# rainerzufalldererste/limg

Measured on AMD Instinct MI355X. Metric: encode Mpixels/s, 8K RGBA (limg_encode3d_test-equivalent: all 11 planes stored), higher is better.
Workload: dtype u8/i32 integer stage + f32 float stage (bit-exact vs the reference's strict SSE build)

## Files before the change

### limg_amd/csrc/limg_hip_device.h

```cpp
#ifndef LIMG_HIP_DEVICE_H
#define LIMG_HIP_DEVICE_H

#include "limg_hip_wave.h"
#include "limg_rsqrt_x86_table.h"

#include <float.h>

namespace limg_hip
{
  namespace
  {
    __device__ __attribute__((aligned(16))) const unsigned short d_rsqrt_x86_tab[2048] = LIMG_RSQRT_X86_TAB_INIT;

    enum : uint32_t { kZeroA = 1u, kZeroB = 2u, kZeroC = 4u, kValid = 8u };

    template <int CTRL, int ROWMASK>
    __device__ __forceinline__ int dpp(int oldv, int v) { return __builtin_amdgcn_update_dpp(oldv, v, CTRL, ROWMASK, 0xF, false); }

    __device__ __forceinline__ uint32_t wave_sum(uint32_t x)
    {
      int v = (int)x;
      v += dpp<0xB1, 0xF>(0, v);
      v += dpp<0x4E, 0xF>(0, v);
      v += dpp<0x141, 0xF>(0, v);
      v += dpp<0x140, 0xF>(0, v);
      v += dpp<0x142, 0xA>(0, v);
      v += dpp<0x143, 0xC>(0, v);
      return (uint32_t)__builtin_amdgcn_readlane(v, 63);
    }

    __device__ __forceinline__ int sgpr(int v) { return __builtin_amdgcn_readfirstlane(v); }
    __device__ __forceinline__ float sgprf(float v) { return __int_as_float(__builtin_amdgcn_readfirstlane(__float_as_int(v))); }

    template <int CH>
    __device__ __forceinline__ float dpps(const float a[4], const float b[4])
    {
      const float p0 = a[0] * b[0], p1 = a[1] * b[1], p2 = a[2] * b[2];
      const float p3 = CH == 4 ? a[3] * b[3] : 0.0f;
      return (p0 + p1) + (p2 + p3);
    }

    __device__ __forceinline__ void px_to_float(uint32_t px, float f[4])
    {
      f[0] = (float)(px & 0xFF); f[1] = (float)((px >> 8) & 0xFF); f[2] = (float)((px >> 16) & 0xFF); f[3] = (float)(px >> 24);
    }

    __device__ __forceinline__ int cvt_rne(float x) { return (int)__builtin_rintf(x); }
    __device__ __forceinline__ uint32_t cvt_u8_rne_sat(float x) { uint32_t r; asm("v_cvt_pk_u8_f32 %0, %1, 0, 0" : "=v"(r) : "v"(x)); return r; }

    __device__ __forceinline__ void store_v(float *V, int lane, const float v[4])
    {
      *reinterpret_cast<float4 *>(V + lane * 4) = make_float4(v[0], v[1], v[2], v[3]);
    }

    struct RecU
    {
      int nA[3], nB[3], nC[3], mA[3], mB[3], mC[3];
    };

    __device__ __forceinline__ uint32_t trial_error(const uint32_t px, const uint32_t fA, const uint32_t fB, const uint32_t fC, const RecU &r, const uint32_t sA,
                                                    const uint32_t sB, const uint32_t sC)
    {
      const uint32_t dA = (fA >> sA) * shift_mul(sA), dB = (fB >> sB) * shift_mul(sB), dC = (fC >> sC) * shift_mul(sC);
      uint32_t dsq[3];
#pragma unroll
      for (int c = 0; c < 3; c++)
      {
        const int nA = sA > 7 ? 0 : r.nA[c], nB = sB > 7 ? 0 : r.nB[c], nC = sC > 7 ? 0 : r.nC[c];
        const int mA = r.mA[c], mB = sB > 7 ? 128 : r.mB[c], mC = sC > 7 ? 128 : r.mC[c];
        int est = ((int)(dA * (uint32_t)nA + (uint32_t)mA) >> 8) + ((int)(dB * (uint32_t)nB + (uint32_t)mB) >> 8) + ((int)(dC * (uint32_t)nC + (uint32_t)mC) >> 8);
        est = est < 0 ? 0 : (est > 255 ? 255 : est);
        const int d = (int)((px >> (8 * c)) & 0xFF) - est;
        dsq[c] = (uint32_t)(d * d);
      }
      const bool low_red = (int)dsq[0] < 0x4000;
      return dsq[0] * (low_red ? 2u : 3u) + dsq[2] * (low_red ? 3u : 2u) + dsq[1] * 4u;
    }

    __device__ __forceinline__ bool trial(const uint32_t px, const uint32_t fA, const uint32_t fB, const uint32_t fC, const RecU &r, const uint32_t sA,
                                          const uint32_t sB, const uint32_t sC, const bool active, const uint32_t maxPixel32, const uint64_t maxBlockN,
                                          uint32_t &blockError)
// ... 291 lines not shown
```

### limg_amd/csrc/limg_hip_encode.hip

```cpp
#include "limg_hip_context.h"
#include "limg_search_table_accurate.h"

using namespace limg_hip;

namespace limg_hip
{
  Partition partition(size_t sizeY, int poolThreads)
  {
    Partition pt = { 1, 0 };
    if (poolThreads <= 0) return pt;
    size_t thread_count = (size_t)poolThreads * 4;
    size_t y_range = ((sizeY / kBlock) / thread_count) * kBlock;
    if (y_range == 0)
    {
      thread_count = (size_t)poolThreads;
      y_range = ((sizeY / kBlock) / thread_count) * kBlock;
    }
    if (y_range == 0) return pt;
    pt.chainCount = (uint32_t)thread_count;
    pt.chainRows = (uint32_t)(y_range / kBlock);
    return pt;
  }

  limg_hip_result encode_stats(const EncodeJob &e)
// ... 38 lines not shown
      e[5] = mul[a]; e[6] = mul[b]; e[7] = mul[cc];
    }
    static_assert((size_t)LIMG_SEARCH_ACC_STATES * 32u < (1u << 24), "offsets leave bits 24..26 free");
    for (size_t i = 0; i < (size_t)LIMG_SEARCH_ACC_STATES; i++)
    {
      uint32_t *e = &wide[i * 8];
      if (e[0] >> 31) continue;
      for (int k = 1; k <= 2; k++)
      {
        const uint32_t *n = &wide[(e[k] / 32u) * 8];
        uint32_t mask = 0;
        if (!(n[0] >> 31)) mask = ((n[0] & 31u) != (e[0] & 31u) ? 1u : 0u) | (n[3] != e[3] ? 2u : 0u) | (n[4] != e[4] ? 4u : 0u);
        e[k] |= mask << 24;
      }
    }
    limg_hip_result r = c->accTable.ensure(wide.size() * 4);
    if (r != limg_hip_success) return r;
    if (hipMemcpy(c->accTable.p, wide.data(), wide.size() * 4, hipMemcpyHostToDevice) != hipSuccess) { c->accTable.release(); return limg_hip_error_Generic; }
    return limg_hip_success;
  }

  limg_hip_result ensure_pipe_events(limg_hip_context *c, size_t n)
  {
    if (!c->fitStream) HIP_TRY(hipStreamCreateWithFlags(&c->fitStream, hipStreamNonBlocking));
    while (c->pipeEvents.size() < n)
    {
      hipEvent_t e;
      HIP_TRY(hipEventCreateWithFlags(&e, hipEventDisableTiming));
      c->pipeEvents.push_back(e);
    }
    return limg_hip_success;
  }

  limg_hip_result encode_height_ragged(limg_hip_context *c, const uint32_t *dIn, size_t sizeX, size_t sizeY, int hasAlpha, const limg_hip_encode3d_info *dInfo,
                                       const limg_hip_compact_out *compact, uint32_t errorFactor, int poolThreads, int fast, hipStream_t stream, const EncodeExtra &x);

  limg_hip_result encode_params(EncodeJob &e, const uint32_t *dIn, const limg_hip_compact_out *compact, uint32_t errorFactor, int poolThreads, int fast)
  {
    limg_hip_context *const c = e.c;
    const EncodeExtra &x = e.x;
    const limg_hip_encode3d_info *const dInfo = e.dInfo;
    const size_t sizeX = e.sizeX, sizeY = e.sizeY, batchCount = x.batchCount;
    const ImageIO *const batch = x.batch;
    EncodeParams &p = e.p;
    memset(&p, 0, sizeof(p));
    p.io.in = dIn;
    p.sizeX = (uint32_t)sizeX; p.sizeY = (uint32_t)sizeY;
    p.blocksX = (uint32_t)((sizeX + kBlock - 1) / kBlock);
    p.blocksY = (uint32_t)((sizeY + kBlock - 1) / kBlock);
    p.stripsX = (p.blocksX + kStripBlocks - 1) / kStripBlocks;
    const uint64_t maxPixel = (uint64_t)0x6 * (errorFactor / 2) * 7, maxBlock = (uint64_t)0x4 * (errorFactor / 2) * 7;
    p.maxPixel32 = maxPixel > 0xFFFFFFFFull ? 0xFFFFFFFFu : (uint32_t)maxPixel;
    p.maxBlock = maxBlock;
    { const uint64_t lim = (maxBlock * 64ull + 15ull) >> 4; p.blockLimitFull = lim > 0xFFFFFFFFull ? 0xFFFFFFFFu : (uint32_t)lim; }
    p.crushBits = errorFactor != 0;
    p.fast = fast != 0;
    p.accTable = nullptr;
    if (!p.fast && p.crushBits)
    {
      limg_hip_result ra = ensure_accurate_table(c);
      if (ra != limg_hip_success) return ra;
      p.accTable = (const uint32_t *)c->accTable.p;
    }
    const bool forced = c->opt.forced_shift[0] >= 0 && c->opt.forced_shift[0] <= 8 && c->opt.forced_shift[1] >= 0 && c->opt.forced_shift[1] <= 8 &&
                        c->opt.forced_shift[2] >= 0 && c->opt.forced_shift[2] <= 8;
    for (int i = 0; i < 3; i++) p.forced[i] = forced ? c->opt.forced_shift[i] : -1;
    p.floatFast = (c->opt.float_mode == 1 && !x.fitOnly) ? 1 : 0;
    p.recordLimit = TOPT(c, record_limit) > 0 ? TOPT(c, record_limit) - 1 : 2700;
    const Partition pt = e.pt = x.part ? *x.part : partition(sizeY, poolThreads);
    p.chainCount = pt.chainCount; p.chainRows = pt.chainRows;

    p.batchCount = (uint32_t)batchCount;
    p.imageStrips = p.stripsX * p.blocksY;
    e.blocks = (size_t)p.blocksX * p.blocksY * batchCount; e.strips = (size_t)p.stripsX * p.blocksY * batchCount;
    const size_t scratchRows = x.scratchRows > (size_t)p.blocksY * batchCount ? x.scratchRows : (size_t)p.blocksY * batchCount;
    const size_t scratchBlocks = scratchRows * p.blocksX, scratchStrips = scratchRows * p.stripsX;
    const size_t blockOff = x.scratchRow0 * p.blocksX, stripOff = x.scratchRow0 * p.stripsX;
    limg_hip_result r;
    if (compact && compact->pRecords) p.records = compact->pRecords + blockOff;
    else { if ((r = c->records.ensure(scratchBlocks * sizeof(limg_hip_block_record))) != limg_hip_success) return r; p.records = (limg_hip_block_record *)c->records.p + blockOff; }
    if (compact && compact->pShifts) p.shifts = compact->pShifts + blockOff;
    else { if ((r = c->shifts.ensure(scratchBlocks * 4)) != limg_hip_success) return r; p.shifts = (uint32_t *)c->shifts.p + blockOff; }
    if ((r = c->invN.ensure(scratchBlocks * 16)) != limg_hip_success) return r;
    p.invN = (float *)c->invN.p + blockOff * 4;
    if ((r = c->stripCalls.ensure(scratchStrips * 4)) != limg_hip_success) return r;
    if ((r = c->stripBase.ensure(scratchStrips * 4)) != limg_hip_success) return r;
    p.stripCalls = (uint32_t *)c->stripCalls.p + stripOff; p.stripBase = (uint32_t *)c->stripBase.p + stripOff;
    const bool fullPlanes = e.fullPlanes;
    p.storePlanes = dInfo != nullptr;
    p.fullPlanes = fullPlanes;
    p.streamRaw = x.streamRaw && !fullPlanes;
    p.stripWords = (x.streamRaw && !fullPlanes) ? x.stripWords : nullptr;
    p.fitOnly = x.fitOnly && !dInfo;
    if (dInfo) p.io.info = *dInfo;
    p.vecIn = (sizeX % 4 == 0) && (((uintptr_t)dIn) & 15u) == 0;
    p.vecPlanes = 0;
    if (dInfo && fullPlanes && sizeX % 4 == 0)
    {
      uintptr_t bits = 0;
      const void *const *pp = reinterpret_cast<const void *const *>(dInfo);
      for (int i = 1; i < 8; i++) bits |= (uintptr_t)pp[i];
      p.vecPlanes = (bits & 15u) == 0;
    }
    p.vecFactors8 = dInfo && (sizeX % 8 == 0) && ((((uintptr_t)dInfo->pFactorsA) | ((uintptr_t)dInfo->pFactorsB) | ((uintptr_t)dInfo->pFactorsC)) & 7u) == 0;
    p.vecDecoded = dInfo && fullPlanes && (sizeX % 4 == 0) && (((uintptr_t)dInfo->pDecoded) & 15u) == 0;
    p.vecFactors = dInfo && (sizeX % 16 == 0) && ((((uintptr_t)dInfo->pFactorsA) | ((uintptr_t)dInfo->pFactorsB) | ((uintptr_t)dInfo->pFactorsC)) & 15u) == 0;
    if (batchCount > 1)
// ... 384 lines not shown
```

### limg_amd/csrc/limg_hip_internal.h

```cpp
#ifndef LIMG_HIP_INTERNAL_H
#define LIMG_HIP_INTERNAL_H

#include <hip/hip_runtime.h>
#include <stdint.h>

#include <type_traits>

#include "../../include/limg_hip.h"
#include "limg_hip_blocked_host.h"

namespace limg_hip
{
  constexpr int kBlock = 8;
  constexpr int kStripBlocks = 32;
  constexpr int kThreads = 256;
  constexpr int kWaves = 4;
  constexpr int kBlocksPerWave = 8;
  constexpr uint64_t kDitherSeed = 0xCA7F00D15BADF00DULL;

  struct ImageIO
  {
    const uint32_t *in;
    limg_hip_encode3d_info info;
  };

  struct EncodeParams
  {
    ImageIO io;
    const ImageIO *batch;
    uint32_t batchCount, imageStrips;
    uint32_t sizeX, sizeY, blocksX, blocksY, stripsX;
    uint32_t maxPixel32;
    uint64_t maxBlock;
    uint32_t blockLimitFull;
    int32_t crushBits, fast;
    const uint32_t *accTable;
    int32_t forced[3];
    int32_t recordLimit;
    uint32_t chainCount, chainRows;
    limg_hip_block_record *records;
    float *invN;
    uint32_t *shifts;
    uint32_t *stripCalls;
    uint32_t *stripBase;
    uint32_t *stripWords;
    int32_t storePlanes;
    int32_t fullPlanes;
    const uint8_t *noise;
    uint32_t noiseLast;
    unsigned long long *desc;
    uint32_t *ticket;
    int32_t zeroLookback;
    uint32_t *timeout;
#ifdef LIMG_HIP_TEST_HOOKS
    uint32_t lookbackSpins;
    uint32_t testBaseErrStrip;
    uint32_t testSkipStrip;
#endif
    uint8_t *park;
    int32_t compactOut;
    int32_t streamRaw;
    int32_t fitOnly;
    unsigned long long *chainCallsOut;
    const unsigned long long *chainBase;
    int32_t fitPrio;
    int32_t prefit;
    int32_t floatFast;
    int32_t vecIn;
    int32_t vecPlanes;
    int32_t vecFactors;
    int32_t vecFactors8;
    int32_t vecDecoded;
  };

  struct StreamParams
  {
    uint32_t sizeX, sizeY, blocksX, blocksY, nBlocks, nTiles, channels, errorFactor, flags;
    const uint8_t *fac[3];
    const limg_hip_block_record *records;
    const uint32_t *shifts;
    uint8_t *stream;
    uint32_t *tileBase;
    uint32_t *stripWords;
    uint32_t stripsX, nStrips, nWaves;
  };

  struct StreamImage
  {
// ... 163 lines not shown
```

### limg_amd/csrc/limg_hip_kernels.hip

```cpp
#include "limg_hip_search.h"
#include "limg_hip_phase_f.h"
#include "limg_hip_float_pixel.h"
#include "limg_hip_lookback.h"

namespace limg_hip
{
  namespace
  {
    constexpr int kPrioE = 2;


    constexpr int kLdsStrip = 0, kLdsV = kLdsStrip + 8 * kRowDw * 4, kLdsVBytes = kWaves * kBatch * kVDw * 4;
    constexpr int kLdsBlk = kLdsV + kLdsVBytes, kLdsCalls = kLdsBlk + kStripBlocks * 192, kLdsTotal = kLdsCalls + 32;
    static_assert(kLdsTotal <= 32768 - 16, "5 workgroups per CU");
    struct LdsLayout { int v, blk, calls, trialc, total; };
    constexpr int kTrialConstDw = 20;
    template <bool PREFIT> __device__ __host__ constexpr LdsLayout lds_layout()
    {
      if (!PREFIT) return LdsLayout{ kLdsV, kLdsBlk, kLdsCalls, kLdsV, kLdsTotal };
      const int v = kLdsStrip + 8 * kRowDw * 4, blk = v + kFacBytes, calls = blk + kStripBlocks * 192, tc = calls + 32, e = tc + kStripBlocks * kTrialConstDw * 4;
      const int f = kLdsStrip + kPhaseFBytes + kStripBlocks * 48 + 16;
      return LdsLayout{ v, blk, calls, tc, e > f ? e : f };
    }
    static_assert(lds_layout<true>().total <= 163840 / 6, "6 workgroups per CU with the float stage in its own kernel");
// ... 354 lines not shown
      uint32_t *s_queue = s_calls + 4;
      if (tid == 0) *s_queue = 0;
      __syncthreads();

      uint8_t *stage = reinterpret_cast<uint8_t *>(s_V);
      uint32_t waveCalls = 0;

      auto grab = [&]() -> uint32_t { uint32_t v = 0; if (lane == 0) v = atomicAdd(s_queue, 1u); return (uint32_t)sgpr((int)v); };
      uint32_t sbNext = grab();
#pragma unroll 1
      for (;;)
      {
        const uint32_t sb = sbNext;
        if (sb >= (uint32_t)kStripBlocks) break;
        uint32_t qv = 0;
        if (lane == 0) qv = atomicAdd(s_queue, 1u);
        const uint32_t bx = strip * kStripBlocks + sb;
        if (bx >= p.blocksX) { sbNext = (uint32_t)sgpr((int)qv); continue; }
        const uint32_t rx = min(p.sizeX - bx * kBlock, (uint32_t)kBlock), n = rx * ry;
        BlkF *const blkE = s_blk + sb;
        uint32_t lx, ly;
        if (rx == 8) { lx = lane & 7; ly = lane >> 3; }
        else { const uint32_t l = (uint32_t)lane < n ? (uint32_t)lane : 0u; ly = l / rx; lx = l - ly * rx; }
        uint32_t px = s_strip[ly * kRowDw + sb * kBlock + lx];
        const bool active = (uint32_t)lane < n;
        px = active ? px : 0u;
        const BlkE *be = reinterpret_cast<const BlkE *>(blkE);

        uint32_t fA, fB, fC;
        {
          const V4 pv = px_to_v4(px);
          const V4 nA = ld4(be->nrm[0]), mnA = ld4(be->off[0]);
          const float fa = dp4<CH, FAST>(pv - mnA, nA) * be->invN[0];
          fA = cvt_u8_rne_sat(255.0f * fa);
          const V4 nB = ld4(be->nrm[1]), ofB = ld4(be->off[1]);
          V4 est = mnA + nA * fa;
          const float fb = dp4<CH, FAST>((pv - est) - ofB, nB) * be->invN[1];
          fB = cvt_u8_rne_sat(255.0f * fb);
          const V4 nC = ld4(be->nrm[2]), ofC = ld4(be->off[2]);
          est = est + nB * fb;
          const float fc = dp4<CH, FAST>((pv - est) - ofC, nC) * be->invN[2];
          fC = cvt_u8_rne_sat(255.0f * fc);
        }

        uint32_t shift[3] = { 0, 0, 0 };
        if (p.forced[0] >= 0)
        {
          shift[0] = (uint32_t)p.forced[0]; shift[1] = (uint32_t)p.forced[1]; shift[2] = (uint32_t)p.forced[2];
        }
        else if (p.crushBits)
        {
          const uint64_t maxBlockN = p.maxBlock * (uint64_t)n;
          uint32_t blockLimit = p.blockLimitFull;
          if (n != 64)
          {
            const uint64_t lim64 = (maxBlockN + 15ull) >> 4;
            blockLimit = (uint32_t)sgpr((int)(lim64 > 0xFFFFFFFFull ? 0xFFFFFFFFu : (uint32_t)lim64));
          }
          const bool big = ((uint32_t)sgpr((int)blkE->flags) & kBig) != 0;
          if (!big)
          {
            TrialState t;
            t.fA = fA; t.fB = fB; t.fC = fC;
            const uint32_t R = px & 0xFF, G = (px >> 8) & 0xFF;
            t.hiRG = (R + 0x8000u) | ((G + 0x8000u) << 16);
            t.loRG = (R + 0x8000u - 255u) | ((G + 0x8000u - 255u) << 16);
            t.pxB = (int)((px >> 16) & 0xFF);
            t.pxBlo = t.pxB - 255;
            if (PREFIT)
            {
              const int *tc = s_trialc + sb * kTrialConstDw;
#pragma unroll
              for (int c = 0; c < 3; c++)
              {
                t.nA[c] = tc[c]; t.nB[c] = tc[3 + c]; t.nC[c] = tc[6 + c];
                t.mA[c] = tc[9 + c]; t.mB[c] = tc[12 + c]; t.mC[c] = tc[15 + c];
              }
            }
            else
            {
#pragma unroll
              for (int c = 0; c < 3; c++)
              {
                const int loA = blkE->rec[c], hiA = blkE->rec[4 + c], loB = blkE->rec[8 + c], hiB = blkE->rec[12 + c], loC = blkE->rec[16 + c], hiC = blkE->rec[20 + c];
                t.nA[c] = loA - hiA; t.nB[c] = loB - hiB; t.nC[c] = loC - hiC;
                t.mA[c] = term_const(0, c, loA); t.mB[c] = term_const(1, c, loB); t.mC[c] = term_const(2, c, loC);
              }
            }
            t.mA[0] += (int)(R << 8); t.mA[1] += (int)(G << 8); t.mA[2] += t.pxB << 8;
            if (!ACC)
            {
              if (n == 64) search_fast_automaton<true>(t, true, p.maxPixel32, blockLimit, shift);
              else search_fast_automaton<false>(t, active, p.maxPixel32, blockLimit, shift);
            }
            else
            {
              if (n == 64) search_accurate_automaton<true>(t, true, p.maxPixel32, blockLimit, p.accTable, shift);
              else search_accurate_automaton<false>(t, active, p.maxPixel32, blockLimit, p.accTable, shift);
            }
          }
          else
          {
            const uint32_t packed = (uint32_t)sgpr((int)search_generic(px, fA, fB, fC, blkE->rec, active, p.maxPixel32, maxBlockN, !ACC));
            shift[0] = packed & 0xFF; shift[1] = (packed >> 8) & 0xFF; shift[2] = (packed >> 16) & 0xFF;
          }
        }

        const uint32_t calls = (((shift[0] & 7u) + 7u) >> 3) + (((shift[1] & 7u) + 7u) >> 3) + (((shift[2] & 7u) + 7u) >> 3);
        waveCalls += calls;
        if (p.stripWords)
        {
          uint32_t words = 0;
#pragma unroll
          for (int k = 0; k < 3; k++)
          {
            const uint32_t sk = shift[k];
            if (sk < 8u) words += 8u - sk;
            else if (CH == 4 && sgpr((int)blkE->rec[8 * k + 3]) != sgpr((int)blkE->rec[8 * k + 7])) words += 8u;
          }
          waveCalls += words << 8;
        }

        const size_t bi = (size_t)byS * p.blocksX + bx;
        const uint32_t word = shift[0] | (shift[1] << 8) | (shift[2] << 16) | (calls << 24);
        if (lane == 0)
        {
          if (!PERSIST || p.compactOut) p.shifts[bi] = word;
          if (PERSIST) reinterpret_cast<uint32_t *>(park + kParkShift)[sb] = word;
        }
        if (p.storePlanes && active)
        {
          const uint32_t o = ly * kFacRow + sb * kBlock + lx;
          stage[o] = (uint8_t)fA; stage[kFacPlane + o] = (uint8_t)fB; stage[2 * kFacPlane + o] = (uint8_t)fC;
        }
        sbNext = (uint32_t)sgpr((int)qv);
      }
      if (lane == 0) s_calls[wave] = waveCalls;
      __syncthreads();
      if (tid == 0)
      {
        const uint32_t aggAll = s_calls[0] + s_calls[1] + s_calls[2] + s_calls[3];
        const uint32_t agg = aggAll & 0xFFu;
        if (p.stripWords) p.stripWords[id] = aggAll >> 8;
        if (PERSIST)
        {
          uint32_t headId = head0;
// ... 337 lines not shown
```

### limg_amd/csrc/limg_hip_search.h

```cpp
#ifndef LIMG_HIP_SEARCH_H
#define LIMG_HIP_SEARCH_H

#include "limg_hip_device.h"
#include "limg_search_table.h"

namespace limg_hip
{
  namespace
  {
    struct __attribute__((aligned(32))) SearchEntry { uint32_t w[8]; };
    __constant__ SearchEntry d_search_tab[LIMG_SEARCH_STATES] = LIMG_SEARCH_TABLE_INIT;

    typedef short short2_t __attribute__((ext_vector_type(2)));
    typedef unsigned short ushort2_t __attribute__((ext_vector_type(2)));
    __device__ __forceinline__ constexpr int term_bias(int factor) { return factor == 2 ? 0x2000 : 0x3000; }
    __device__ __forceinline__ int term_const(int f, int c, int lo) { return 255 - ((lo << 8) + 128) + (c < 2 ? (term_bias(f) << 8) : 0); }

    struct TrialState
    {
      uint32_t fA, fB, fC;
      uint32_t loRG, hiRG;
      int pxB, pxBlo;
      int nA[3], nB[3], nC[3];
      int mA[3], mB[3], mC[3];
// ... 25 lines not shown
    }

    template <bool FULL>
    __device__ __forceinline__ uint32_t trial_pixel_error(const TrialState &t, const bool active)
    {
      const uint32_t dRG = t.tA_RG + t.tB_RG + t.tC_RG;
      const int dBraw = t.tA_B + t.tB_B + t.tC_B;
      ushort2_t eu = __builtin_bit_cast(ushort2_t, dRG);
      eu = __builtin_elementwise_max(eu, __builtin_bit_cast(ushort2_t, t.loRG));
      eu = __builtin_elementwise_min(eu, __builtin_bit_cast(ushort2_t, t.hiRG));
      int dB = med3_i32(dBraw, t.pxBlo, t.pxB);
      const ushort2_t sq = eu * eu;
      const uint32_t sqB = (uint32_t)mul_i24(dB, dB);
      const bool low_red = sq.x < 0x4000;
      const uint32_t half = __builtin_amdgcn_udot2(sq, __builtin_bit_cast(ushort2_t, 0x00020001u), sqB, false);
      const uint32_t extra = low_red ? sqB : (__builtin_bit_cast(uint32_t, sq) & 0xFFFFu);
      uint32_t err = (half << 1) + extra;
      if (!FULL) err = active ? err : 0u;
      return err;
    }

    typedef unsigned int uint8s_t __attribute__((ext_vector_type(8)));
    __device__ __forceinline__ uint8s_t sload8(const SearchEntry *base, uint32_t byteOffset)
    {
      uint8s_t v;
      asm volatile("s_load_dwordx8 %0, %1, %2\n\ts_waitcnt lgkmcnt(0)" : "=&s"(v) : "s"(base), "s"(byteOffset) : "memory");
      return v;
    }

    struct TermSet { uint32_t rg; int b; };
    __device__ __forceinline__ constexpr TermSet terms_shift8(int factor) { return TermSet{ (uint32_t)term_bias(factor) * 0x10001u, 0 }; }
    template <uint32_t S, uint32_t MUL>
    __device__ __forceinline__ TermSet hot_terms(const uint32_t f, const int n[3], const int m[3])
    {
      static_assert(S <= 8 && (S >= 4 || MUL == (1u << S)), "MUL is shift_mul(S)");
      int t0, t1, t2;
      if constexpr (S == 8) { t0 = m[0]; t1 = m[1]; t2 = m[2]; }
      else
      {
        uint32_t d;
        if constexpr (S < 4) d = f & ~((1u << S) - 1u);
        else asm("v_mul_u32_u24 %0, %2, %1" : "=v"(d) : "v"(f >> S), "n"(MUL));
        t0 = mad_i24((int)d, n[0], m[0]); t1 = mad_i24((int)d, n[1], m[1]); t2 = mad_i24((int)d, n[2], m[2]);
      }
      TermSet r;
      r.rg = __builtin_amdgcn_perm((uint32_t)t1, (uint32_t)t0, 0x06050201u);
      r.b = t2 >> 8;
      return r;
    }
    __device__ __forceinline__ bool hot_trial(TrialState &t, const TermSet &A, const TermSet &B, const TermSet &C, const uint32_t maxPixel32, const uint32_t blockLimit)
    {
      t.tA_RG = A.rg; t.tA_B = A.b; t.tB_RG = B.rg; t.tB_B = B.b; t.tC_RG = C.rg; t.tC_B = C.b;
      const uint32_t err = trial_pixel_error<true>(t, true);
      return __builtin_amdgcn_ballot_w64(err > maxPixel32) == 0ull && wave_sum(err) < blockLimit;
    }
#include "limg_search_hot.h"

    template <bool FULL>
    __device__ __forceinline__ void search_fast_automaton(TrialState &t, const bool active, const uint32_t maxPixel32, const uint32_t blockLimit, uint32_t shift[3])
    {
      const SearchEntry *tab = d_search_tab;
      uint8s_t e;
      if constexpr (FULL)
      {
        uint32_t off;
        if (search_hot(t, maxPixel32, blockLimit, shift, off)) return;
        asm volatile("" : "+s"(tab));
        e = sload8(tab, off);
      }
      else
      {
        asm volatile("" : "+s"(tab));
        constexpr uint32_t root[8] = LIMG_SEARCH_ROOT;
        rebuild_A(t, root[0] & 31u, root[5]);
        rebuild_B(t, root[3], root[6]);
        rebuild_C(t, root[4], root[7]);
        e = uint8s_t{ root[0] & ~0xE0u, root[1], root[2], root[3], root[4], root[5], root[6], root[7] };
      }
      while (!(e[0] >> 31))
      {
        if (e[0] & 0x20u) rebuild_A(t, e[0] & 31u, e[5]);
        if (e[0] & 0x40u) rebuild_B(t, e[3], e[6]);
        if (e[0] & 0x80u) rebuild_C(t, e[4], e[7]);
        const uint32_t err = trial_pixel_error<FULL>(t, active);
        uint32_t off;
        if (__builtin_amdgcn_ballot_w64(err > maxPixel32) != 0ull) off = e[2];
        else off = (wave_sum(err) < blockLimit) ? e[1] : e[2];
        e = sload8(tab, off);
      }
      shift[0] = e[0] & 31u; shift[1] = e[3]; shift[2] = e[4];
    }

    template <bool FULL>
    __device__ __forceinline__ void search_accurate_automaton(TrialState &t, const bool active, const uint32_t maxPixel32, const uint32_t blockLimit, const uint32_t *table,
                                                              uint32_t shift[3])
    {
      const SearchEntry *tab = reinterpret_cast<const SearchEntry *>(table);
      uint32_t bestA = 0, bestB = 0, bestC = 0, minBe = 0xFFFFFFFFu;
      {
        constexpr uint32_t root[8] = LIMG_SEARCH_ROOT;
        rebuild_A(t, root[0] & 31u, root[5]);
        rebuild_B(t, root[3], root[6]);
        rebuild_C(t, root[4], root[7]);
      }
      uint8s_t e = sload8(tab, 0u);
      constexpr uint32_t rootT[8] = LIMG_SEARCH_ROOT;
      uint32_t mask = ((e[0] & 31u) != (rootT[0] & 31u) ? 1u : 0u) | (e[3] != rootT[3] ? 2u : 0u) | (e[4] != rootT[4] ? 4u : 0u);
      while (!(e[0] >> 31))
      {
        const uint32_t a = e[0] & 31u;
        if (mask & 1u) rebuild_A(t, a, e[5]);
        if (mask & 2u) rebuild_B(t, e[3], e[6]);
        if (mask & 4u) rebuild_C(t, e[4], e[7]);
        const uint32_t err = trial_pixel_error<FULL>(t, active);
        uint32_t off = e[2];
        if (__builtin_amdgcn_ballot_w64(err > maxPixel32) == 0ull)
        {
          const uint32_t be = wave_sum(err);
          if (be < blockLimit)
          {
            off = e[1];
            if (!(e[0] & 0x20u) || be < minBe) { bestA = a; bestB = e[3]; bestC = e[4]; minBe = be; }
          }
        }
        mask = off >> 24;
        e = sload8(tab, off & 0xFFFFFFu);
      }
      shift[0] = bestA; shift[1] = bestB; shift[2] = bestC;
    }

    __device__ __attribute__((noinline)) uint32_t search_generic(uint32_t px, uint32_t fA, uint32_t fB, uint32_t fC, const int16_t *rec , bool active,
                                                                 uint32_t maxPixel32, uint64_t maxBlockN, bool fast)
    {
      RecU r;
#pragma unroll
      for (int c = 0; c < 3; c++)
      {
        const int loA = rec[c], hiA = rec[4 + c], loB = rec[8 + c], hiB = rec[12 + c], loC = rec[16 + c], hiC = rec[20 + c];
        r.nA[c] = sgpr(hiA - loA); r.nB[c] = sgpr(hiB - loB); r.nC[c] = sgpr(hiC - loC);
        r.mA[c] = sgpr((int)(((uint32_t)loA << 8) + 128u)); r.mB[c] = sgpr((int)(((uint32_t)loB << 8) + 128u)); r.mC[c] = sgpr((int)(((uint32_t)loC << 8) + 128u));
// ... 12 lines not shown
```

### limg_amd/csrc/limg_search_hot.h

```cpp
#ifndef LIMG_SEARCH_HOT_H
#define LIMG_SEARCH_HOT_H
#define LIMG_SEARCH_HOT_STATES 45
__device__ __forceinline__ bool search_hot(TrialState &t, const uint32_t maxPixel32, const uint32_t blockLimit, uint32_t shift[3], uint32_t &off)
{
  const TermSet tA4_0 = hot_terms<4u, 17u>(t.fA, t.nA, t.mA);
  const TermSet tB5_0 = hot_terms<5u, 36u>(t.fB, t.nB, t.mB);
  const TermSet tC6_0 = hot_terms<6u, 85u>(t.fC, t.nC, t.mC);
  if (hot_trial(t, tA4_0, tB5_0, tC6_0, maxPixel32, blockLimit))
  {
    const TermSet tA5_1 = hot_terms<5u, 36u>(t.fA, t.nA, t.mA);
    if (hot_trial(t, tA5_1, terms_shift8(1), terms_shift8(2), maxPixel32, blockLimit))
    { shift[0] = 5u; shift[1] = 8u; shift[2] = 8u; return true; }
    else
    {
      const TermSet tB6_3 = hot_terms<6u, 85u>(t.fB, t.nB, t.mB);
      if (hot_trial(t, tA4_0, tB6_3, terms_shift8(2), maxPixel32, blockLimit))
      {
        if (hot_trial(t, tA4_0, terms_shift8(1), terms_shift8(2), maxPixel32, blockLimit))
        { t.cA = 4u; t.cB = 8u; t.cC = 8u; off = 0x00a0u; return false; }
        else
        {
          const TermSet tA6_23 = hot_terms<6u, 85u>(t.fA, t.nA, t.mA);
          if (hot_trial(t, tA6_23, tB6_3, terms_shift8(2), maxPixel32, blockLimit))
          {
            if (hot_trial(t, tA6_23, terms_shift8(1), terms_shift8(2), maxPixel32, blockLimit))
            { t.cA = 6u; t.cB = 8u; t.cC = 8u; off = 0x00c0u; return false; }
            else
            {
              const TermSet tA8_25 = hot_terms<8u, 256u>(t.fA, t.nA, t.mA);
              if (hot_trial(t, tA8_25, tB6_3, terms_shift8(2), maxPixel32, blockLimit))
              { t.cA = 8u; t.cB = 6u; t.cC = 8u; off = 0x0180u; return false; }
              else
              {
                if (hot_trial(t, tA8_25, terms_shift8(1), tC6_0, maxPixel32, blockLimit))
                { t.cA = 8u; t.cB = 8u; t.cC = 6u; off = 0x0220u; return false; }
                else
                {
                  const TermSet tB7_27 = hot_terms<7u, 255u>(t.fB, t.nB, t.mB);
                  if (hot_trial(t, tA6_23, tB7_27, terms_shift8(2), maxPixel32, blockLimit))
                  { t.cA = 6u; t.cB = 7u; t.cC = 8u; off = 0x0380u; return false; }
                  else
                  {
                    const TermSet tA7_31 = hot_terms<7u, 255u>(t.fA, t.nA, t.mA);
                    if (hot_trial(t, tA7_31, tB6_3, terms_shift8(2), maxPixel32, blockLimit))
                    { t.cA = 7u; t.cB = 6u; t.cC = 8u; off = 0x0400u; return false; }
                    else
                    { shift[0] = 6u; shift[1] = 6u; shift[2] = 8u; return true; }
                  }
                }
              }
            }
          }
          else
          {
            if (hot_trial(t, tA6_23, terms_shift8(1), tC6_0, maxPixel32, blockLimit))
            { t.cA = 6u; t.cB = 8u; t.cC = 6u; off = 0x0480u; return false; }
            else
            {
              const TermSet tA8_47 = hot_terms<8u, 256u>(t.fA, t.nA, t.mA);
              if (hot_trial(t, tA8_47, tB6_3, terms_shift8(2), maxPixel32, blockLimit))
              { t.cA = 8u; t.cB = 6u; t.cC = 8u; off = 0x0180u; return false; }
              else
              {
                if (hot_trial(t, tA8_47, terms_shift8(1), tC6_0, maxPixel32, blockLimit))
                { t.cA = 8u; t.cB = 8u; t.cC = 6u; off = 0x0220u; return false; }
                else
                {
                  const TermSet tB7_49 = hot_terms<7u, 255u>(t.fB, t.nB, t.mB);
                  if (hot_trial(t, tA4_0, tB7_49, terms_shift8(2), maxPixel32, blockLimit))
                  { t.cA = 4u; t.cB = 7u; t.cC = 8u; off = 0x0640u; return false; }
                  else
                  {
                    if (hot_trial(t, tA5_1, tB6_3, terms_shift8(2), maxPixel32, blockLimit))
                    {
                      if (hot_trial(t, tA5_1, tB7_49, terms_shift8(2), maxPixel32, blockLimit))
                      { shift[0] = 5u; shift[1] = 7u; shift[2] = 8u; return true; }
                      else
                      { shift[0] = 5u; shift[1] = 6u; shift[2] = 8u; return true; }
                    }
                    else
                    { shift[0] = 4u; shift[1] = 6u; shift[2] = 8u; return true; }
                  }
                }
              }
            }
          }
        }
      }
      else
      {
        if (hot_trial(t, tA4_0, tB5_0, terms_shift8(2), maxPixel32, blockLimit))
        { t.cA = 4u; t.cB = 5u; t.cC = 8u; off = 0x0740u; return false; }
        else
        {
          const TermSet tB7_96 = hot_terms<7u, 255u>(t.fB, t.nB, t.mB);
          const TermSet tC5_96 = hot_terms<5u, 36u>(t.fC, t.nC, t.mC);
          if (hot_trial(t, tA4_0, tB7_96, tC5_96, maxPixel32, blockLimit))
          { t.cA = 4u; t.cB = 7u; t.cC = 5u; off = 0x0c20u; return false; }
          else
          {
            const TermSet tA6_112 = hot_terms<6u, 85u>(t.fA, t.nA, t.mA);
            const TermSet tB4_112 = hot_terms<4u, 17u>(t.fB, t.nB, t.mB);
            const TermSet tC7_112 = hot_terms<7u, 255u>(t.fC, t.nC, t.mC);
            if (hot_trial(t, tA6_112, tB4_112, tC7_112, maxPixel32, blockLimit))
            { t.cA = 6u; t.cB = 4u; t.cC = 7u; off = 0x0c60u; return false; }
            else
            {
              const TermSet tC4_113 = hot_terms<4u, 17u>(t.fC, t.nC, t.mC);
              if (hot_trial(t, tA6_112, tB6_3, tC4_113, maxPixel32, blockLimit))
              { t.cA = 6u; t.cB = 6u; t.cC = 4u; off = 0x0e40u; return false; }
              else
              {
                if (hot_trial(t, tA6_112, terms_shift8(1), tC6_0, maxPixel32, blockLimit))
                { t.cA = 6u; t.cB = 8u; t.cC = 6u; off = 0x0480u; return false; }
                else
                {
                  const TermSet tA8_138 = hot_terms<8u, 256u>(t.fA, t.nA, t.mA);
                  if (hot_trial(t, tA8_138, tB6_3, terms_shift8(2), maxPixel32, blockLimit))
                  { t.cA = 8u; t.cB = 6u; t.cC = 8u; off = 0x0180u; return false; }
                  else
                  {
                    if (hot_trial(t, tA8_138, terms_shift8(1), tC6_0, maxPixel32, blockLimit))
                    { t.cA = 8u; t.cB = 8u; t.cC = 6u; off = 0x0220u; return false; }
                    else
                    {
                      if (hot_trial(t, tA4_0, tB5_0, tC7_112, maxPixel32, blockLimit))
                      { t.cA = 4u; t.cB = 5u; t.cC = 7u; off = 0x11a0u; return false; }
                      else
                      {
                        if (hot_trial(t, tA5_1, tB5_0, tC6_0, maxPixel32, blockLimit))
                        {
                          if (hot_trial(t, tA5_1, tB5_0, tC7_112, maxPixel32, blockLimit))
                          { shift[0] = 5u; shift[1] = 5u; shift[2] = 7u; return true; }
                          else
                          { shift[0] = 5u; shift[1] = 5u; shift[2] = 6u; return true; }
                        }
                        else
                        { shift[0] = 4u; shift[1] = 5u; shift[2] = 6u; return true; }
                      }
                    }
                  }
                }
              }
            }
          }
        }
      }
    }
  }
  else
  {
    const TermSet tA2_148 = hot_terms<2u, 4u>(t.fA, t.nA, t.mA);
    const TermSet tB4_148 = hot_terms<4u, 17u>(t.fB, t.nB, t.mB);
    const TermSet tC5_148 = hot_terms<5u, 36u>(t.fC, t.nC, t.mC);
    if (hot_trial(t, tA2_148, tB4_148, tC5_148, maxPixel32, blockLimit))
    {
      const TermSet tC7_149 = hot_terms<7u, 255u>(t.fC, t.nC, t.mC);
      if (hot_trial(t, tA2_148, tB4_148, tC7_149, maxPixel32, blockLimit))
      { t.cA = 2u; t.cB = 4u; t.cC = 7u; off = 0x12c0u; return false; }
      else
      {
        const TermSet tB6_378 = hot_terms<6u, 85u>(t.fB, t.nB, t.mB);
        const TermSet tC4_378 = hot_terms<4u, 17u>(t.fC, t.nC, t.mC);
        if (hot_trial(t, tA2_148, tB6_378, tC4_378, maxPixel32, blockLimit))
        { t.cA = 2u; t.cB = 6u; t.cC = 4u; off = 0x2f60u; return false; }
        else
        {
          if (hot_trial(t, tA2_148, terms_shift8(1), tC6_0, maxPixel32, blockLimit))
          { t.cA = 2u; t.cB = 8u; t.cC = 6u; off = 0x18e0u; return false; }
          else
          {
            const TermSet tB2_412 = hot_terms<2u, 4u>(t.fB, t.nB, t.mB);
            if (hot_trial(t, tA4_0, tB2_412, terms_shift8(2), maxPixel32, blockLimit))
            { t.cA = 4u; t.cB = 2u; t.cC = 8u; off = 0x2500u; return false; }
            else
            {
              if (hot_trial(t, tA4_0, tB4_148, tC4_378, maxPixel32, blockLimit))
              {
                if (hot_trial(t, tA4_0, tB4_148, tC6_0, maxPixel32, blockLimit))
                { t.cA = 4u; t.cB = 4u; t.cC = 6u; off = 0x2700u; return false; }
                else
                {
                  if (hot_trial(t, tA4_0, tB6_378, tC4_378, maxPixel32, blockLimit))
                  { t.cA = 4u; t.cB = 6u; t.cC = 4u; off = 0x2a40u; return false; }
                  else
                  {
                    if (hot_trial(t, tA4_0, terms_shift8(1), tC6_0, maxPixel32, blockLimit))
                    { t.cA = 4u; t.cB = 8u; t.cC = 6u; off = 0x1460u; return false; }
                    else
                    {
                      const TermSet tA6_417 = hot_terms<6u, 85u>(t.fA, t.nA, t.mA);
                      if (hot_trial(t, tA6_417, tB4_148, terms_shift8(2), maxPixel32, blockLimit))
                      { t.cA = 6u; t.cB = 4u; t.cC = 8u; off = 0x1620u; return false; }
                      else
                      {
                        if (hot_trial(t, tA6_417, tB6_378, tC4_378, maxPixel32, blockLimit))
                        { t.cA = 6u; t.cB = 6u; t.cC = 4u; off = 0x0e40u; return false; }
                        else
                        {
                          if (hot_trial(t, tA6_417, terms_shift8(1), tC6_0, maxPixel32, blockLimit))
                          { t.cA = 6u; t.cB = 8u; t.cC = 6u; off = 0x0480u; return false; }
                          else
                          {
                            const TermSet tA8_420 = hot_terms<8u, 256u>(t.fA, t.nA, t.mA);
                            if (hot_trial(t, tA8_420, tB6_378, terms_shift8(2), maxPixel32, blockLimit))
                            { t.cA = 8u; t.cB = 6u; t.cC = 8u; off = 0x0180u; return false; }
                            else
                            {
                              if (hot_trial(t, tA8_420, terms_shift8(1), tC6_0, maxPixel32, blockLimit))
                              { t.cA = 8u; t.cB = 8u; t.cC = 6u; off = 0x0220u; return false; }
                              else
                              {
                                if (hot_trial(t, tA4_0, tB4_148, tC5_148, maxPixel32, blockLimit))
                                {
                                  if (hot_trial(t, tA4_0, tB5_0, tC5_148, maxPixel32, blockLimit))
                                  {
                                    const TermSet tA5_424 = hot_terms<5u, 36u>(t.fA, t.nA, t.mA);
                                    if (hot_trial(t, tA5_424, tB5_0, tC5_148, maxPixel32, blockLimit))
                                    { shift[0] = 5u; shift[1] = 5u; shift[2] = 5u; return true; }
                                    else
                                    { shift[0] = 4u; shift[1] = 5u; shift[2] = 5u; return true; }
                                  }
                                  else
                                  {
                                    const TermSet tA5_427 = hot_terms<5u, 36u>(t.fA, t.nA, t.mA);
                                    if (hot_trial(t, tA5_427, tB4_148, tC5_148, maxPixel32, blockLimit))
                                    { t.cA = 5u; t.cB = 4u; t.cC = 5u; off = 0x3580u; return false; }
                                    else
                                    {
                                      if (hot_trial(t, tA5_427, tB5_0, tC4_378, maxPixel32, blockLimit))
                                      { t.cA = 5u; t.cB = 5u; t.cC = 4u; off = 0x35e0u; return false; }
                                      else
                                      { shift[0] = 4u; shift[1] = 4u; shift[2] = 5u; return true; }
                                    }
                                  }
                                }
                                else
                                { t.cA = 4u; t.cB = 4u; t.cC = 5u; off = 0x3640u; return false; }
                              }
                            }
                          }
                        }
                      }
                    }
                  }
                }
              }
              else
              { t.cA = 4u; t.cB = 4u; t.cC = 4u; off = 0x3780u; return false; }
            }
          }
        }
      }
    }
    else
    { t.cA = 2u; t.cB = 4u; t.cC = 5u; off = 0x3880u; return false; }
  }
}
#endif
```

Measured before the change: 54590.

## Add ballot-count early-reject screens before wave sum in hot search trials

Adds a cheap pre-screen to many hot-path search trials. It counts the lanes whose error meets a per-K threshold (limit/K) with a ballot and popcount, and rejects the trial when K or more lanes exceed it, since their sum must then reach the limit. This aims to skip the DPP reduction on failing trials. Separately, the wave-sum comparison now uses a ballot on lane 63 instead of readlane. The screen adds extra ballots and popcounts on trials that pass, and its benefit depends on how often the trials that were screened actually fail.

```diff
diff --git a/limg_amd/csrc/limg_hip_device.h b/limg_amd/csrc/limg_hip_device.h
--- a/limg_amd/csrc/limg_hip_device.h
+++ b/limg_amd/csrc/limg_hip_device.h
@@ -27,6 +27,20 @@
       v += dpp<0x142, 0xA>(0, v);
       v += dpp<0x143, 0xC>(0, v);
       return (uint32_t)__builtin_amdgcn_readlane(v, 63);
+    }
+
+    __device__ __forceinline__ bool wave_sum_below(uint32_t x, uint32_t limit)
+    {
+      int v = (int)x;
+      v += dpp<0xB1, 0xF>(0, v);
+      v += dpp<0x4E, 0xF>(0, v);
+      v += dpp<0x141, 0xF>(0, v);
+      v += dpp<0x140, 0xF>(0, v);
+      v += dpp<0x142, 0xA>(0, v);
+      v += dpp<0x143, 0xC>(0, v);
+      uint32_t hi = (uint32_t)(__builtin_amdgcn_ballot_w64((uint32_t)v < limit) >> 32);
+      asm volatile("" : "+s"(hi));
+      return (int32_t)hi < 0;
     }
 
     __device__ __forceinline__ int sgpr(int v) { return __builtin_amdgcn_readfirstlane(v); }
diff --git a/limg_amd/csrc/limg_hip_encode.hip b/limg_amd/csrc/limg_hip_encode.hip
--- a/limg_amd/csrc/limg_hip_encode.hip
+++ b/limg_amd/csrc/limg_hip_encode.hip
@@ -114,7 +114,8 @@
     const uint64_t maxPixel = (uint64_t)0x6 * (errorFactor / 2) * 7, maxBlock = (uint64_t)0x4 * (errorFactor / 2) * 7;
     p.maxPixel32 = maxPixel > 0xFFFFFFFFull ? 0xFFFFFFFFu : (uint32_t)maxPixel;
     p.maxBlock = maxBlock;
-    { const uint64_t lim = (maxBlock * 64ull + 15ull) >> 4; p.blockLimitFull = lim > 0xFFFFFFFFull ? 0xFFFFFFFFu : (uint32_t)lim; }
+    p.blockLimitFull = block_sum_limit(maxBlock, 64);
+    for (int i = 0; i < 4; i++) p.sumScreenT[i] = sum_screen_threshold(p.blockLimitFull, 8u << i);
     p.crushBits = errorFactor != 0;
     p.fast = fast != 0;
     p.accTable = nullptr;
diff --git a/limg_amd/csrc/limg_hip_internal.h b/limg_amd/csrc/limg_hip_internal.h
--- a/limg_amd/csrc/limg_hip_internal.h
+++ b/limg_amd/csrc/limg_hip_internal.h
@@ -8,6 +8,7 @@
 
 #include "../../include/limg_hip.h"
 #include "limg_hip_blocked_host.h"
+#include "limg_hip_sum_screen.h"
 
 namespace limg_hip
 {
@@ -34,6 +35,7 @@
     uint64_t maxBlock;
     uint32_t blockLimitFull;
     int32_t crushBits, fast;
+    uint32_t sumScreenT[4];
     const uint32_t *accTable;
     int32_t forced[3];
     int32_t recordLimit;
diff --git a/limg_amd/csrc/limg_hip_kernels.hip b/limg_amd/csrc/limg_hip_kernels.hip
--- a/limg_amd/csrc/limg_hip_kernels.hip
+++ b/limg_amd/csrc/limg_hip_kernels.hip
@@ -430,11 +430,7 @@
         {
           const uint64_t maxBlockN = p.maxBlock * (uint64_t)n;
           uint32_t blockLimit = p.blockLimitFull;
-          if (n != 64)
-          {
-            const uint64_t lim64 = (maxBlockN + 15ull) >> 4;
-            blockLimit = (uint32_t)sgpr((int)(lim64 > 0xFFFFFFFFull ? 0xFFFFFFFFu : (uint32_t)lim64));
-          }
+          if (n != 64) blockLimit = (uint32_t)sgpr((int)block_sum_limit(p.maxBlock, n));
           const bool big = ((uint32_t)sgpr((int)blkE->flags) & kBig) != 0;
           if (!big)
           {
@@ -468,8 +464,9 @@
             t.mA[0] += (int)(R << 8); t.mA[1] += (int)(G << 8); t.mA[2] += t.pxB << 8;
             if (!ACC)
             {
-              if (n == 64) search_fast_automaton<true>(t, true, p.maxPixel32, blockLimit, shift);
-              else search_fast_automaton<false>(t, active, p.maxPixel32, blockLimit, shift);
+              const uint32_t sumT[4] = { p.sumScreenT[0], p.sumScreenT[1], p.sumScreenT[2], p.sumScreenT[3] };
+              if (n == 64) search_fast_automaton<true>(t, true, p.maxPixel32, blockLimit, sumT, shift);
+              else search_fast_automaton<false>(t, active, p.maxPixel32, blockLimit, sumT, shift);
             }
             else
             {
diff --git a/limg_amd/csrc/limg_hip_search.h b/limg_amd/csrc/limg_hip_search.h
--- a/limg_amd/csrc/limg_hip_search.h
+++ b/limg_amd/csrc/limg_hip_search.h
@@ -101,19 +101,49 @@
     {
       t.tA_RG = A.rg; t.tA_B = A.b; t.tB_RG = B.rg; t.tB_B = B.b; t.tC_RG = C.rg; t.tC_B = C.b;
       const uint32_t err = trial_pixel_error<true>(t, true);
-      return __builtin_amdgcn_ballot_w64(err > maxPixel32) == 0ull && wave_sum(err) < blockLimit;
+      return __builtin_amdgcn_ballot_w64(err > maxPixel32) == 0ull && wave_sum_below(err, blockLimit);
+    }
+    __device__ __forceinline__ uint32_t lane_count(const uint64_t mask) { uint32_t c; asm("s_bcnt1_i32_b64 %0, %1" : "=s"(c) : "s"(mask) : "scc"); return c; }
+    template <int K>
+    __device__ __forceinline__ bool sum_screen(const uint32_t err, const uint32_t TK) { return lane_count(__builtin_amdgcn_ballot_w64(err >= TK)) >= (uint32_t)K; }
+    template <int K>
+    __device__ __forceinline__ bool hot_trial_after(TrialState &t, const TermSet &A, const TermSet &B, const TermSet &C, const uint32_t maxPixel32, const uint32_t blockLimit,
+                                                    const uint32_t TK)
+    {
+      t.tA_RG = A.rg; t.tA_B = A.b; t.tB_RG = B.rg; t.tB_B = B.b; t.tC_RG = C.rg; t.tC_B = C.b;
+      const uint32_t err = trial_pixel_error<true>(t, true);
+      return __builtin_amdgcn_ballot_w64(err > maxPixel32) == 0ull && !sum_screen<K>(err, TK) && wave_sum_below(err, blockLimit);
+    }
+    template <int K>
+    __device__ __forceinline__ bool hot_trial_first(TrialState &t, const TermSet &A, const TermSet &B, const TermSet &C, const uint32_t maxPixel32, const uint32_t blockLimit,
+                                                    const uint32_t TK)
+    {
+      t.tA_RG = A.rg; t.tA_B = A.b; t.tB_RG = B.rg; t.tB_B = B.b; t.tC_RG = C.rg; t.tC_B = C.b;
+      const uint32_t err = trial_pixel_error<true>(t, true);
+      return !sum_screen<K>(err, TK) && __builtin_amdgcn_ballot_w64(err > maxPixel32) == 0ull && wave_sum_below(err, blockLimit);
+    }
+    template <int K>
+    __device__ __forceinline__ bool hot_trial_two(TrialState &t, const TermSet &A, const TermSet &B, const TermSet &C, const uint32_t maxPixel32, const uint32_t blockLimit,
+                                                  const uint32_t TK, const uint32_t TH)
+    {
+      t.tA_RG = A.rg; t.tA_B = A.b; t.tB_RG = B.rg; t.tB_B = B.b; t.tC_RG = C.rg; t.tC_B = C.b;
+      const uint32_t err = trial_pixel_error<true>(t, true);
+      if (__builtin_amdgcn_ballot_w64(err > maxPixel32) != 0ull) return false;
+      const uint32_t nLo = lane_count(__builtin_amdgcn_ballot_w64(err >= TK)), nHi = lane_count(__builtin_amdgcn_ballot_w64(err >= TH));
+      return 3u * nHi + nLo < (uint32_t)K && wave_sum_below(err, blockLimit);
     }
 #include "limg_search_hot.h"
 
     template <bool FULL>
-    __device__ __forceinline__ void search_fast_automaton(TrialState &t, const bool active, const uint32_t maxPixel32, const uint32_t blockLimit, uint32_t shift[3])
+    __device__ __forceinline__ void search_fast_automaton(TrialState &t, const bool active, const uint32_t maxPixel32, const uint32_t blockLimit, const uint32_t sumT[4],
+                                                          uint32_t shift[3])
     {
       const SearchEntry *tab = d_search_tab;
       uint8s_t e;
       if constexpr (FULL)
       {
         uint32_t off;
-        if (search_hot(t, maxPixel32, blockLimit, shift, off)) return;
+        if (search_hot(t, maxPixel32, blockLimit, sumT, shift, off)) return;
         asm volatile("" : "+s"(tab));
         e = sload8(tab, off);
       }
@@ -134,7 +164,7 @@
         const uint32_t err = trial_pixel_error<FULL>(t, active);
         uint32_t off;
         if (__builtin_amdgcn_ballot_w64(err > maxPixel32) != 0ull) off = e[2];
-        else off = (wave_sum(err) < blockLimit) ? e[1] : e[2];
+        else off = wave_sum_below(err, blockLimit) ? e[1] : e[2];
         e = sload8(tab, off);
       }
       shift[0] = e[0] & 31u; shift[1] = e[3]; shift[2] = e[4];
diff --git a/limg_amd/csrc/limg_hip_sum_screen.h b/limg_amd/csrc/limg_hip_sum_screen.h
--- /dev/null
+++ b/limg_amd/csrc/limg_hip_sum_screen.h
@@ -0,0 +1,22 @@
+#ifndef LIMG_HIP_SUM_SCREEN_H
+#define LIMG_HIP_SUM_SCREEN_H
+
+#include <stdint.h>
+
+#if defined(__HIPCC__)
+#define LIMG_HIP_HD __host__ __device__
+#else
+#define LIMG_HIP_HD
+#endif
+
+namespace limg_hip
+{
+  LIMG_HIP_HD inline uint32_t block_sum_limit(uint64_t maxBlock, uint32_t n)
+  {
+    const uint64_t lim = (maxBlock * (uint64_t)n + 15ull) >> 4;
+    return lim > 0xFFFFFFFFull ? 0xFFFFFFFFu : (uint32_t)lim;
+  }
+  LIMG_HIP_HD inline uint32_t sum_screen_threshold(uint32_t limit, uint32_t k) { return (uint32_t)(((uint64_t)limit + k - 1u) / k); }
+}
+
+#endif
diff --git a/limg_amd/csrc/limg_search_hot.h b/limg_amd/csrc/limg_search_hot.h
--- a/limg_amd/csrc/limg_search_hot.h
+++ b/limg_amd/csrc/limg_search_hot.h
@@ -1,7 +1,7 @@
 #ifndef LIMG_SEARCH_HOT_H
 #define LIMG_SEARCH_HOT_H
 #define LIMG_SEARCH_HOT_STATES 45
-__device__ __forceinline__ bool search_hot(TrialState &t, const uint32_t maxPixel32, const uint32_t blockLimit, uint32_t shift[3], uint32_t &off)
+__device__ __forceinline__ bool search_hot(TrialState &t, const uint32_t maxPixel32, const uint32_t blockLimit, const uint32_t sumT[4], uint32_t shift[3], uint32_t &off)
 {
   const TermSet tA4_0 = hot_terms<4u, 17u>(t.fA, t.nA, t.mA);
   const TermSet tB5_0 = hot_terms<5u, 36u>(t.fB, t.nB, t.mB);
@@ -28,21 +28,21 @@
             else
             {
               const TermSet tA8_25 = hot_terms<8u, 256u>(t.fA, t.nA, t.mA);
-              if (hot_trial(t, tA8_25, tB6_3, terms_shift8(2), maxPixel32, blockLimit))
+              if (hot_trial_first<32>(t, tA8_25, tB6_3, terms_shift8(2), maxPixel32, blockLimit, sumT[2]))
               { t.cA = 8u; t.cB = 6u; t.cC = 8u; off = 0x0180u; return false; }
               else
               {
-                if (hot_trial(t, tA8_25, terms_shift8(1), tC6_0, maxPixel32, blockLimit))
+                if (hot_trial_first<32>(t, tA8_25, terms_shift8(1), tC6_0, maxPixel32, blockLimit, sumT[2]))
                 { t.cA = 8u; t.cB = 8u; t.cC = 6u; off = 0x0220u; return false; }
                 else
                 {
                   const TermSet tB7_27 = hot_terms<7u, 255u>(t.fB, t.nB, t.mB);
-                  if (hot_trial(t, tA6_23, tB7_27, terms_shift8(2), maxPixel32, blockLimit))
+                  if (hot_trial_first<32>(t, tA6_23, tB7_27, terms_shift8(2), maxPixel32, blockLimit, sumT[2]))
                   { t.cA = 6u; t.cB = 7u; t.cC = 8u; off = 0x0380u; return false; }
                   else
                   {
                     const TermSet tA7_31 = hot_terms<7u, 255u>(t.fA, t.nA, t.mA);
-                    if (hot_trial(t, tA7_31, tB6_3, terms_shift8(2), maxPixel32, blockLimit))
+                    if (hot_trial_first<32>(t, tA7_31, tB6_3, terms_shift8(2), maxPixel32, blockLimit, sumT[2]))
                     { t.cA = 7u; t.cB = 6u; t.cC = 8u; off = 0x0400u; return false; }
                     else
                     { shift[0] = 6u; shift[1] = 6u; shift[2] = 8u; return true; }
@@ -53,27 +53,27 @@
           }
           else
           {
-            if (hot_trial(t, tA6_23, terms_shift8(1), tC6_0, maxPixel32, blockLimit))
+            if (hot_trial_two<64>(t, tA6_23, terms_shift8(1), tC6_0, maxPixel32, blockLimit, sumT[3], sumT[1]))
             { t.cA = 6u; t.cB = 8u; t.cC = 6u; off = 0x0480u; return false; }
             else
             {
               const TermSet tA8_47 = hot_terms<8u, 256u>(t.fA, t.nA, t.mA);
-              if (hot_trial(t, tA8_47, tB6_3, terms_shift8(2), maxPixel32, blockLimit))
+              if (hot_trial_first<32>(t, tA8_47, tB6_3, terms_shift8(2), maxPixel32, blockLimit, sumT[2]))
               { t.cA = 8u; t.cB = 6u; t.cC = 8u; off = 0x0180u; return false; }
               else
               {
-                if (hot_trial(t, tA8_47, terms_shift8(1), tC6_0, maxPixel32, blockLimit))
+                if (hot_trial_first<16>(t, tA8_47, terms_shift8(1), tC6_0, maxPixel32, blockLimit, sumT[1]))
                 { t.cA = 8u; t.cB = 8u; t.cC = 6u; off = 0x0220u; return false; }
                 else
                 {
                   const TermSet tB7_49 = hot_terms<7u, 255u>(t.fB, t.nB, t.mB);
-                  if (hot_trial(t, tA4_0, tB7_49, terms_shift8(2), maxPixel32, blockLimit))
+                  if (hot_trial_first<32>(t, tA4_0, tB7_49, terms_shift8(2), maxPixel32, blockLimit, sumT[2]))
                   { t.cA = 4u; t.cB = 7u; t.cC = 8u; off = 0x0640u; return false; }
                   else
                   {
                     if (hot_trial(t, tA5_1, tB6_3, terms_shift8(2), maxPixel32, blockLimit))
                     {
-                      if (hot_trial(t, tA5_1, tB7_49, terms_shift8(2), maxPixel32, blockLimit))
+                      if (hot_trial_first<32>(t, tA5_1, tB7_49, terms_shift8(2), maxPixel32, blockLimit, sumT[2]))
                       { shift[0] = 5u; shift[1] = 7u; shift[2] = 8u; return true; }
                       else
                       { shift[0] = 5u; shift[1] = 6u; shift[2] = 8u; return true; }
@@ -95,23 +95,23 @@
         {
           const TermSet tB7_96 = hot_terms<7u, 255u>(t.fB, t.nB, t.mB);
           const TermSet tC5_96 = hot_terms<5u, 36u>(t.fC, t.nC, t.mC);
-          if (hot_trial(t, tA4_0, tB7_96, tC5_96, maxPixel32, blockLimit))
+          if (hot_trial_first<32>(t, tA4_0, tB7_96, tC5_96, maxPixel32, blockLimit, sumT[2]))
           { t.cA = 4u; t.cB = 7u; t.cC = 5u; off = 0x0c20u; return false; }
           else
           {
             const TermSet tA6_112 = hot_terms<6u, 85u>(t.fA, t.nA, t.mA);
             const TermSet tB4_112 = hot_terms<4u, 17u>(t.fB, t.nB, t.mB);
             const TermSet tC7_112 = hot_terms<7u, 255u>(t.fC, t.nC, t.mC);
-            if (hot_trial(t, tA6_112, tB4_112, tC7_112, maxPixel32, blockLimit))
+            if (hot_trial_first<32>(t, tA6_112, tB4_112, tC7_112, maxPixel32, blockLimit, sumT[2]))
             { t.cA = 6u; t.cB = 4u; t.cC = 7u; off = 0x0c60u; return false; }
             else
             {
               const TermSet tC4_113 = hot_terms<4u, 17u>(t.fC, t.nC, t.mC);
-              if (hot_trial(t, tA6_112, tB6_3, tC4_113, maxPixel32, blockLimit))
+              if (hot_trial_two<64>(t, tA6_112, tB6_3, tC4_113, maxPixel32, blockLimit, sumT[3], sumT[1]))
               { t.cA = 6u; t.cB = 6u; t.cC = 4u; off = 0x0e40u; return false; }
               else
               {
-                if (hot_trial(t, tA6_112, terms_shift8(1), tC6_0, maxPixel32, blockLimit))
+                if (hot_trial_first<32>(t, tA6_112, terms_shift8(1), tC6_0, maxPixel32, blockLimit, sumT[2]))
                 { t.cA = 6u; t.cB = 8u; t.cC = 6u; off = 0x0480u; return false; }
                 else
                 {
@@ -124,13 +124,13 @@
                     { t.cA = 8u; t.cB = 8u; t.cC = 6u; off = 0x0220u; return false; }
                     else
                     {
-                      if (hot_trial(t, tA4_0, tB5_0, tC7_112, maxPixel32, blockLimit))
+                      if (hot_trial_first<32>(t, tA4_0, tB5_0, tC7_112, maxPixel32, blockLimit, sumT[2]))
                       { t.cA = 4u; t.cB = 5u; t.cC = 7u; off = 0x11a0u; return false; }
                       else
                       {
                         if (hot_trial(t, tA5_1, tB5_0, tC6_0, maxPixel32, blockLimit))
                         {
-                          if (hot_trial(t, tA5_1, tB5_0, tC7_112, maxPixel32, blockLimit))
+                          if (hot_trial_first<32>(t, tA5_1, tB5_0, tC7_112, maxPixel32, blockLimit, sumT[2]))
                           { shift[0] = 5u; shift[1] = 5u; shift[2] = 7u; return true; }
                           else
                           { shift[0] = 5u; shift[1] = 5u; shift[2] = 6u; return true; }
@@ -156,22 +156,22 @@
     if (hot_trial(t, tA2_148, tB4_148, tC5_148, maxPixel32, blockLimit))
     {
       const TermSet tC7_149 = hot_terms<7u, 255u>(t.fC, t.nC, t.mC);
-      if (hot_trial(t, tA2_148, tB4_148, tC7_149, maxPixel32, blockLimit))
+      if (hot_trial_first<32>(t, tA2_148, tB4_148, tC7_149, maxPixel32, blockLimit, sumT[2]))
       { t.cA = 2u; t.cB = 4u; t.cC = 7u; off = 0x12c0u; return false; }
       else
       {
         const TermSet tB6_378 = hot_terms<6u, 85u>(t.fB, t.nB, t.mB);
         const TermSet tC4_378 = hot_terms<4u, 17u>(t.fC, t.nC, t.mC);
-        if (hot_trial(t, tA2_148, tB6_378, tC4_378, maxPixel32, blockLimit))
+        if (hot_trial_first<16>(t, tA2_148, tB6_378, tC4_378, maxPixel32, blockLimit, sumT[1]))
         { t.cA = 2u; t.cB = 6u; t.cC = 4u; off = 0x2f60u; return false; }
         else
         {
-          if (hot_trial(t, tA2_148, terms_shift8(1), tC6_0, maxPixel32, blockLimit))
+          if (hot_trial_first<16>(t, tA2_148, terms_shift8(1), tC6_0, maxPixel32, blockLimit, sumT[1]))
           { t.cA = 2u; t.cB = 8u; t.cC = 6u; off = 0x18e0u; return false; }
           else
           {
             const TermSet tB2_412 = hot_terms<2u, 4u>(t.fB, t.nB, t.mB);
-            if (hot_trial(t, tA4_0, tB2_412, terms_shift8(2), maxPixel32, blockLimit))
+            if (hot_trial_first<16>(t, tA4_0, tB2_412, terms_shift8(2), maxPixel32, blockLimit, sumT[1]))
             { t.cA = 4u; t.cB = 2u; t.cC = 8u; off = 0x2500u; return false; }
             else
             {
@@ -181,24 +181,24 @@
                 { t.cA = 4u; t.cB = 4u; t.cC = 6u; off = 0x2700u; return false; }
                 else
                 {
-                  if (hot_trial(t, tA4_0, tB6_378, tC4_378, maxPixel32, blockLimit))
+                  if (hot_trial_two<64>(t, tA4_0, tB6_378, tC4_378, maxPixel32, blockLimit, sumT[3], sumT[1]))
                   { t.cA = 4u; t.cB = 6u; t.cC = 4u; off = 0x2a40u; return false; }
                   else
                   {
-                    if (hot_trial(t, tA4_0, terms_shift8(1), tC6_0, maxPixel32, blockLimit))
+                    if (hot_trial_first<16>(t, tA4_0, terms_shift8(1), tC6_0, maxPixel32, blockLimit, sumT[1]))
                     { t.cA = 4u; t.cB = 8u; t.cC = 6u; off = 0x1460u; return false; }
                     else
                     {
                       const TermSet tA6_417 = hot_terms<6u, 85u>(t.fA, t.nA, t.mA);
-                      if (hot_trial(t, tA6_417, tB4_148, terms_shift8(2), maxPixel32, blockLimit))
+                      if (hot_trial_first<16>(t, tA6_417, tB4_148, terms_shift8(2), maxPixel32, blockLimit, sumT[1]))
                       { t.cA = 6u; t.cB = 4u; t.cC = 8u; off = 0x1620u; return false; }
                       else
                       {
-                        if (hot_trial(t, tA6_417, tB6_378, tC4_378, maxPixel32, blockLimit))
+                        if (hot_trial_first<32>(t, tA6_417, tB6_378, tC4_378, maxPixel32, blockLimit, sumT[2]))
                         { t.cA = 6u; t.cB = 6u; t.cC = 4u; off = 0x0e40u; return false; }
                         else
                         {
-                          if (hot_trial(t, tA6_417, terms_shift8(1), tC6_0, maxPixel32, blockLimit))
+                          if (hot_trial_first<8>(t, tA6_417, terms_shift8(1), tC6_0, maxPixel32, blockLimit, sumT[0]))
                           { t.cA = 6u; t.cB = 8u; t.cC = 6u; off = 0x0480u; return false; }
                           else
                           {
@@ -228,7 +228,7 @@
                                     { t.cA = 5u; t.cB = 4u; t.cC = 5u; off = 0x3580u; return false; }
                                     else
                                     {
-                                      if (hot_trial(t, tA5_427, tB5_0, tC4_378, maxPixel32, blockLimit))
+                                      if (hot_trial_two<64>(t, tA5_427, tB5_0, tC4_378, maxPixel32, blockLimit, sumT[3], sumT[1]))
                                       { t.cA = 5u; t.cB = 5u; t.cC = 4u; off = 0x35e0u; return false; }
                                       else
                                       { shift[0] = 4u; shift[1] = 4u; shift[2] = 5u; return true; }
```

After: 54980, median of 6. About the same (+0.7%).
